# f1tenth/f1tenth_planning

Hardware: AMD Instinct MI355X
Metric: candidate-trajectory-steps/sec per GPU; p50 plan() latency @4096 egos (higher is better)
Workload: dtype f32 filter + f64 decision

## Files before the change

f1tenth_planning_amd/csrc/k_lattice_refine.hip:

```cpp
#include "lattice_mixed.h"

namespace f1p {

template <int GS>
__device__ __forceinline__ double group_shr1(double v) {
    const long long b = __double_as_longlong(v);
    const int lo = (int)(b & 0xffffffffll), hi = (int)(b >> 32);
    constexpr int ctrl = GS == 16 ? 0x111 : 0x138;
    const int slo = __builtin_amdgcn_update_dpp(0, lo, ctrl, 0xf, 0xf, false), shi = __builtin_amdgcn_update_dpp(0, hi, ctrl, 0xf, 0xf, false);
    return __longlong_as_double(((long long)shi << 32) | (long long)(unsigned int)slo);
}

template <int GS, bool FOOT = false, typename... OB>
__global__ __launch_bounds__(256, 2) void k_lattice_refine(const unsigned int* __restrict__ h_qcount, const RefEntry* __restrict__ h_q, unsigned int h_q_shard_cap, unsigned int h_grid,
                                                           LatticeArgs a, f1p_lattice_cfg cfg, MixArgs mx, OB... obx) {
    extern __shared__ __align__(16) unsigned char lds_raw[];
    constexpr bool OBS = sizeof...(OB) > 0;
    int ka[32];
    warm_kernargs_touch<24 + sizeof(LatticeArgs) + sizeof(f1p_lattice_cfg) + sizeof(MixArgs) + (sizeof(OB) + ... + 0)>(ka);
    constexpr int GPW = 64 / GS;
    constexpr unsigned int WPB = F1P_MIX_REFINE_BLOCK / 64;
    const int tid = threadIdx.x, lane = tid & 63, wave = tid >> 6;
    const int gl = lane & (GS - 1), grp = lane / GS, gbase = lane & ~(GS - 1);
    const unsigned int ngroups_total = h_grid * WPB * GPW;
    const unsigned int g0 = (blockIdx.x * WPB + wave) * GPW + grp;
    const unsigned int sh = (g0 / GPW) % F1P_MIX_QSHARDS, lstride = ngroups_total / F1P_MIX_QSHARDS;
    const unsigned int li_first = (g0 / (GPW * F1P_MIX_QSHARDS)) * GPW + g0 % GPW;
    RefEntry r_first;
    r_first.ok = 0; r_first.e = 0; r_first.c = 0; r_first.gx = 0; r_first.gy = 0; r_first.gth = 0; r_first.cost = 0; r_first.k0 = 0; r_first.dk = 0; r_first.L = 0; r_first.pad = 0;
    unsigned int n = h_qcount[sh * 32u];
    if (li_first < h_q_shard_cap) r_first = h_q[sh * h_q_shard_cap + li_first];
    warm_kernargs_wait(ka, n, r_first.ok);
    const int S_arg = cfg.n_stations;
    if (mx.perm_fill) {
        const int np = F1P_MIX_OREG * mx.perm_rs;
        for (int i = (int)(blockIdx.x * blockDim.x) + tid; i < np; i += (int)(gridDim.x * blockDim.x)) mx.perm_fill[i] = 0;
        if (blockIdx.x == 0 && tid < 2 * F1P_MIX_OREG) mx.ocnt[tid * 32u] = 0u;
    }
    __shared__ double s_gl_wu[16][6];
    __shared__ double s_gl_x[16];
#ifdef F1P_MIX_PHASES
    long long rph[16]; int nrp = 0;
#define F1P_RPH() do { if (nrp < 15) rph[nrp++] = clock64(); } while (0)
#else
#define F1P_RPH() do {} while (0)
#endif
    F1P_RPH();
    const bool collide_on = cfg.check_collision && a.has_grid;
    if (tid < 96) s_gl_wu[tid / 6][tid % 6] = c_gl_wu[tid / 6][tid % 6];
    else if (tid < 112) s_gl_x[tid - 96] = c_gl_x[tid - 96];
    __syncthreads();
    asm volatile("" : "+v"(n), "+v"(r_first.ok));
    for (unsigned int ib = 0, li = li_first; ; ib += ngroups_total, li += lstride) {
#ifdef F1P_MIX_REFINE_LICM
        const int S = S_arg;
#else
        int S = S_arg;
        asm volatile("" : "+s"(S));
#endif
        const int den = S - 1 > 1 ? S - 1 : 1;
        const int sim_m = S - cfg.n_shift - cfg.n_cull;
        double* ncs = reinterpret_cast<double*>(lds_raw) + (size_t)(wave * GPW + grp) * (64 + 4 * (size_t)S);
        double* nsn = ncs + 32;
        double* inc_x = nsn + 32;
        double* inc_y = inc_x + S;
        double* akv = inc_y + S;
        double* simv = akv + S;
        const unsigned int i = sh * mx.q_shard_cap + li;
        const bool live = li < n;
        if (!__any(live)) break;
        RefEntry r = r_first;
        if (ib != 0) {
            r.ok = 0; r.e = 0; r.c = 0; r.gx = 0; r.gy = 0; r.gth = 0; r.cost = 0; r.k0 = 0; r.dk = 0; r.L = 0; r.pad = 0;
            if (li < mx.q_shard_cap) r = mx.q[i];
        }
        if (!live) { r.ok = 0; r.e = a.e0; r.c = 0; }
        F1P_RPH();
        const bool work = live && r.ok != 0;
        const int e = r.e;
        const bool check_occ = collide_on && r.ok != -2;
        EgoXform xf = {};
        if (work && check_occ) xf = mx.xf[e];
        [[maybe_unused]] bool check_disc = false;
        [[maybe_unused]] int n_live = 0;
        [[maybe_unused]] double pace = 0.0;
        [[maybe_unused]] const double* slots = nullptr;
        if constexpr (OBS) {
            const LatObs& ob = lat_obs_arg(obx...);
            if (work && r.ok != -2) {
                n_live = ob.n_live[e]; pace = ob.pace[e]; slots = ob.xf + (size_t)e * (5 * F1P_LATTICE_MAX_OBS);
                check_disc = n_live > 0;
            }
        }
        const double* prev = a.prev_theta ? a.prev_theta + (size_t)e * S : nullptr;
        double pv[4] = {0.0, 0.0, 0.0, 0.0};
        if (work && prev) {
#pragma unroll
            for (int k = 0; k < 4; ++k) { const int q = gl + k * GS; if (q < sim_m) pv[k] = prev[q + cfg.n_shift]; }
        }
        Clothoid cl;
        cl.ok = false; cl.k0 = 0; cl.dk = 0; cl.L = 0;
        G1State g;
        g.r = 0; g.phi0 = 0; g.delta = 0; g.A = 0;
        bool fitting = work && g1_begin(r.gx, r.gy, r.gth, g);
        F1P_RPH();
        double c0 = 0.0;
        bool ok = false;
        for (int it = 0; it < 20 && __any(fitting); ++it) {
            const double fa = g.A, fb = g.delta - g.A, fc = g.phi0;
            const double exc = fabs(fa) + fabs(fb);
            int off = 88, cnt = 32, panels = 1;
            if (exc <= 8.0) { off = 0; cnt = 16; }
            else if (exc <= 14.0) { off = 16; cnt = 20; }
            else if (exc <= 21.0) { off = 36; cnt = 24; }
            else if (exc <= 29.0) { off = 60; cnt = 28; }
            else if (!(exc <= 36.0)) {
                const double pn = __builtin_ceil(exc * (1.0 / 36.0));
                panels = pn <= 1024.0 ? (int)pn : 1024;
            }
            if (!fitting) { cnt = 0; panels = 1; }
            double acc = 0.0;
            const int k = gl < 6 ? gl : gl - 6;
            int max_panels = panels;
            if (__any(panels > 1)) {
#pragma unroll
                for (int m_ = 32; m_ >= 1; m_ >>= 1) { const int o = __shfl_xor(max_panels, m_, 64); max_panels = o > max_panels ? o : max_panels; }
            }
            if (max_panels == 1) {
                const bool rule16 = cnt == 16;
                for (int j = gl; j < cnt; j += GS) {
                    const double tau = rule16 ? s_gl_x[j] : c_gl_x[off + j];
                    const double ph = __builtin_fma(__builtin_fma(fa, tau, fb), tau, fc);
                    double sn, cs;
                    sincos_core(ph, &sn, &cs);
                    ncs[j] = cs; nsn[j] = sn;
                }
                __builtin_amdgcn_s_waitcnt(0xc07f);
                __builtin_amdgcn_wave_barrier();
#ifdef F1P_MIX_PHASES
                if (it == 0) F1P_RPH();
#endif
                if (gl < 12) {
                    const double* v = gl < 6 ? ncs : nsn;
                    if (rule16) {
                        double w[16], u[16];
#pragma unroll
                        for (int j = 0; j < 16; ++j) { w[j] = s_gl_wu[j][k]; u[j] = v[j]; }
#pragma unroll
                        for (int j = 0; j < 16; ++j) acc = __builtin_fma(w[j], u[j], acc);
                    } else {
                        for (int j0 = 0; j0 < cnt; j0 += 4) {
                            const double w0 = c_gl_wu[off + j0][k], w1 = c_gl_wu[off + j0 + 1][k], w2 = c_gl_wu[off + j0 + 2][k], w3 = c_gl_wu[off + j0 + 3][k];
                            const double u0 = v[j0], u1 = v[j0 + 1], u2 = v[j0 + 2], u3 = v[j0 + 3];
                            acc = __builtin_fma(w0, u0, acc); acc = __builtin_fma(w1, u1, acc); acc = __builtin_fma(w2, u2, acc); acc = __builtin_fma(w3, u3, acc);
                        }
                    }
                }
                __builtin_amdgcn_wave_barrier();
            } else {
                const double h = 1.0 / (double)panels;
                for (int p = 0; p < max_panels; ++p) {
                    const bool mine = fitting && p < panels;
                    if (mine && panels == 1) {
                        for (int j = gl; j < cnt; j += GS) {
                            const double tau = c_gl_x[off + j];
                            const double ph = __builtin_fma(__builtin_fma(fa, tau, fb), tau, fc);
                            double sn, cs;
                            sincos_core(ph, &sn, &cs);
                            ncs[j] = cs; nsn[j] = sn;
                        }
                    } else if (mine) {
                        const double t0 = (double)p * h;
                        for (int j = gl; j < cnt; j += GS) {
                            const double tau = __builtin_fma(h, c_gl_x[off + j], t0);
                            const double ph = __builtin_fma(__builtin_fma(fa, tau, fb), tau, fc);
                            double sn, cs;
                            sincos_core(ph, &sn, &cs);
                            const double w = h * c_gl_w[off + j];
                            ncs[j] = w * cs; nsn[j] = w * sn;
                            akv[j] = __builtin_fma(tau, tau, -tau);
                        }
                    }
                    __builtin_amdgcn_s_waitcnt(0xc07f);
                    __builtin_amdgcn_wave_barrier();
                    if (mine && gl < 12) {
                        const double* v = gl < 6 ? ncs : nsn;
                        if (panels == 1) {
                            for (int j = 0; j < cnt; ++j) acc = __builtin_fma(c_gl_wu[off + j][k], v[j], acc);
                        } else {
                            for (int j = 0; j < cnt; ++j) {
                                double t = v[j];
                                for (int q = 0; q < k; ++q) t *= akv[j];
                                acc += t;
                            }
                        }
                    }
                    __builtin_amdgcn_wave_barrier();
                }
            }
            FitMoments m;
#pragma unroll
            for (int q = 0; q < 6; ++q) { m.c[q] = shfl_d(acc, gbase + q); m.s[q] = shfl_d(acc, gbase + 6 + q); }
#ifdef F1P_MIX_PHASES
            if (it == 0) F1P_RPH();
#endif
            if (fitting) {
                const int st = g1_step(m, g, c0);
                if (st != 0) { fitting = false; ok = st > 0; }
            }
        }
        if (ok) cl = g1_finish(g, c0);
        F1P_RPH();
        double cost = __builtin_huge_val();
        const bool run = cl.ok;
        const double k0 = cl.k0, dk = cl.dk, L = run ? cl.L : 1.0;
        const double ds = L / (double)den;
        bool hit = false;
        const bool occ_pass = run && (check_occ || (OBS && check_disc));
        const bool store_inc = run && mx.inc != nullptr && li < mx.inc_cap;
        const bool inc_pass = occ_pass || store_inc;
        double rix[4] = {0.0, 0.0, 0.0, 0.0}, riy[4] = {0.0, 0.0, 0.0, 0.0};
        if (__any(inc_pass)) {
            if (inc_pass) {
                const IntervalCoef ic = interval_setup(k0, dk, L, ds);
                const int per = (S - 1 + GS - 1) / GS, q0 = gl * per, q1 = q0 + per < S - 1 ? q0 + per : S - 1;
                if (!FOOT && per <= 4) {
#pragma unroll
                    for (int k = 0; k < 4; ++k) { rix[k] = 0.0; riy[k] = 0.0; }
                    if (q0 < q1) {
                        PieceState st = piece_state_at(k0, dk, ds, q0, ic);
#pragma unroll
                        for (int k = 0; k < 4; ++k) {
                            if (q0 + k < q1) interval_increment(k0, dk, (double)(q0 + k) * ds, (q0 + k) * ic.nsub, ic, st, rix[k], riy[k]);
                        }
                    }
                } else if (q0 < q1) {
                    PieceState st = piece_state_at(k0, dk, ds, q0, ic);
                    for (int q = q0; q < q1; ++q) {
                        double dx, dy;
                        interval_increment(k0, dk, (double)q * ds, q * ic.nsub, ic, st, dx, dy);
                        inc_x[q] = dx; inc_y[q] = dy;
                    }
                }
            }
            __builtin_amdgcn_s_waitcnt(0xc07f);
            __builtin_amdgcn_wave_barrier();
            F1P_RPH();
            double* gp = store_inc ? mx.inc + ((size_t)sh * mx.inc_cap + li) * 2 * (size_t)S : nullptr;
            double* pos_x = akv; double* pos_y = simv;
            if (inc_pass) {
                const int per = (S - 1 + GS - 1) / GS;
                if (gl == 0) { pos_x[0] = 0.0; pos_y[0] = 0.0; }
                if (!FOOT && per <= 4) {
                    const int nrounds = (S - 1 + per - 1) / per;
                    double xin = 0.0, yin = 0.0, xo = 0.0, yo = 0.0;
                    for (int t = 0; t < nrounds; ++t) {
                        xin = group_shr1<GS>(xo); yin = group_shr1<GS>(yo);
                        xo = xin; yo = yin;
#pragma unroll
                        for (int k = 0; k < 4; ++k) { xo += rix[k]; yo += riy[k]; }
                    }
                    double x = xin, y = yin;
                    const int q0 = gl * per;
#pragma unroll
                    for (int k = 0; k < 4; ++k) {
                        x += rix[k]; y += riy[k];
                        if (k < per && q0 + k < S - 1) { pos_x[q0 + k + 1] = x; pos_y[q0 + k + 1] = y; }
                    }
                } else {
                double x = 0.0, y = 0.0;
                int j0 = 0;
                for (; j0 + 8 <= S - 1; j0 += 8) {
                    double dx[8], dy[8], xs[8], ys[8];
#pragma unroll
                    for (int u = 0; u < 8; ++u) { dx[u] = inc_x[j0 + u]; dy[u] = inc_y[j0 + u]; }
#pragma unroll
                    for (int u = 0; u < 8; ++u) { x += dx[u]; y += dy[u]; xs[u] = x; ys[u] = y; }
                    if (gl == 0) {
#pragma unroll
                        for (int u = 0; u < 8; ++u) { pos_x[j0 + u + 1] = xs[u]; pos_y[j0 + u + 1] = ys[u]; }
                    }
                }
                for (; j0 < S - 1; ++j0) {
                    x += inc_x[j0]; y += inc_y[j0];
                    if (gl == 0) { pos_x[j0 + 1] = x; pos_y[j0 + 1] = y; }
                }
                }
            }
            __builtin_amdgcn_s_waitcnt(0xc07f);
            __builtin_amdgcn_wave_barrier();
            F1P_RPH();
            if (inc_pass) {
                constexpr int NSL = 4;
                for (int qb = 0; qb < S; qb += NSL * GS) {
                    double xs[NSL], ys[NSL];
#pragma unroll
                    for (int k = 0; k < NSL; ++k) { const int q = qb + k * GS + gl; xs[k] = q < S ? pos_x[q] : 0.0; ys[k] = q < S ? pos_y[q] : 0.0; }
                    auto cell = [&](double qx, double qy, uint32_t& word, int& bit) {
                        word = 0xffffffffu; bit = 0;
                        const double lxf = __builtin_floor(__builtin_fma(xf.txx, qx, __builtin_fma(xf.txy, qy, xf.tx0)));
                        const double lyf = __builtin_floor(__builtin_fma(xf.tyx, qx, __builtin_fma(xf.tyy, qy, xf.ty0)));
                        const double gxf = lxf + (double)xf.tile_gx0, gyf = lyf + (double)xf.tile_gy0;
                        if ((gxf >= 0.0) & (gxf < (double)a.grid.w) & (gyf >= 0.0) & (gyf < (double)a.grid.h)) {
                            const int cgx = (int)gxf, cgy = (int)gyf;
                            word = a.grid.bits[(size_t)cgy * a.grid.wwords + (cgx >> 5)];
                            bit = cgx & 31;
                        }
                    };
                    if (gp) {
#pragma unroll
                        for (int k = 0; k < NSL; ++k) { const int q = qb + k * GS + gl; if (q < S) { __builtin_nontemporal_store(xs[k], gp + q); __builtin_nontemporal_store(ys[k], gp + S + q); } }
                    }
                    if (!occ_pass) continue;
                    if constexpr (OBS) {
                        if (check_disc) {
#pragma unroll
                            for (int k = 0; k < NSL; ++k) {
                                const int q = qb + k * GS + gl;
                                if (q < S) hit |= lat_disc_blocked(slots, n_live, xs[k], ys[k], ((double)q * ds) * pace);
                            }
                        }
                        if (!check_occ) continue;
                    }
                    if (!FOOT || mx.n_disc == 0) {
                        uint32_t word[NSL]; int bit[NSL]; bool have[NSL];
#pragma unroll
                        for (int k = 0; k < NSL; ++k) {
                            have[k] = qb + k * GS + gl < S;
                            word[k] = 0u; bit[k] = 0;
                            if (have[k]) cell(xs[k], ys[k], word[k], bit[k]);
                        }
#pragma unroll
                        for (int k = 0; k < NSL; ++k) hit |= have[k] && ((word[k] >> bit[k]) & 1u);
                    } else {
#pragma unroll
                        for (int k = 0; k < NSL; ++k) {
                            const int q = qb + k * GS + gl;
                            if (q < S) {
                                const double sq = (double)q * ds;
                                const double th = sq * (k0 + 0.5 * sq * dk);
                                double sn_h, cs_h;
                                sincos_fast(th, &sn_h, &cs_h);
                                for (int d = 0; d < mx.n_disc; ++d) {
                                    const double o = mx.disc_off[d];
                                    uint32_t word; int bit;
                                    cell(xs[k] + o * cs_h, ys[k] + o * sn_h, word, bit);
                                    hit |= (word >> bit) & 1u;
                                }
                            }
                        }
                    }
                }
            }
            __builtin_amdgcn_s_waitcnt(0xc07f);
            __builtin_amdgcn_wave_barrier();
        }
        F1P_RPH();
        if (run) {
            for (int q = gl; q < S; q += GS) {
                const double s = (double)q * ds;
                akv[q] = fabs(k0 + dk * s);
                double sv = 0.0;
                if (prev && q < sim_m) {
                    const int kq = (q - gl) / GS;
                    const double pq = kq < 4 ? (kq == 0 ? pv[0] : (kq == 1 ? pv[1] : (kq == 2 ? pv[2] : pv[3]))) : prev[q + cfg.n_shift];
                    const double th = s * (k0 + 0.5 * s * dk); const double d = th - pq; sv = d * d;
                }
                simv[q] = sv;
            }
        }
        __builtin_amdgcn_s_waitcnt(0xc07f);
        __builtin_amdgcn_wave_barrier();
        F1P_RPH();
        const unsigned long long hm = __ballot(hit);
        const bool any_hit = ((hm >> gbase) & (GS == 64 ? ~0ull : (1ull << (GS & 63)) - 1ull)) != 0ull;
        if (run) {
            double sumk = 0.0, sim = 0.0;
            {
                int q = 0;
                for (; q + 8 <= S; q += 8) {
                    double v[8];
#pragma unroll
                    for (int u = 0; u < 8; ++u) v[u] = akv[q + u];
#pragma unroll
                    for (int u = 0; u < 8; ++u) sumk += v[u];
                }
                for (; q < S; ++q) sumk += akv[q];
            }
            if (prev) {
                int q = 0;
                for (; q + 8 <= sim_m; q += 8) {
                    double v[8];
#pragma unroll
                    for (int u = 0; u < 8; ++u) v[u] = simv[q + u];
#pragma unroll
                    for (int u = 0; u < 8; ++u) sim += v[u];
                }
                for (; q < sim_m; ++q) sim += simv[q];
            }
            const double maxk = __builtin_fmax(fabs(k0 + dk * (0.0 * ds)), fabs(k0 + dk * ((double)(S - 1) * ds)));
            cost = 0.0;
            cost += cfg.w_length * (1.0 / L);
            cost += cfg.w_max_kappa * maxk;
            cost += cfg.w_mean_kappa * (sumk / (double)S);
            cost += cfg.w_similarity * sim;
            if (any_hit) cost = __builtin_huge_val();
        }
        __builtin_amdgcn_wave_barrier();
        if (work && gl == 0) {
            RefEntry o = r;
            o.cost = cost; o.k0 = cl.k0; o.dk = cl.dk; o.L = cl.L; o.ok = cl.ok ? 1 : 0; o.pad = store_inc ? 1 : 0;
            mx.q[i] = o;
        }
#ifdef F1P_MIX_PHASES
        F1P_RPH();
        if (ib == 0 && live && gl == 0 && mx.dbg_state && (size_t)i * 16 + 16 <= (size_t)a.E * cfg.n_lookahead * cfg.n_width) {
            for (int k = 0; k + 1 < nrp; ++k) mx.dbg_state[(size_t)i * 16 + k] = (int)(rph[k + 1] - rph[k]);
            mx.dbg_state[(size_t)i * 16 + 15] = nrp;
        }
#endif
    }
}

template <int GS, bool FOOT = false>
__global__ __launch_bounds__(256, 2) void k_lattice_refine_cubic(LatticeArgs a, f1p_lattice_cfg cfg, MixArgs mx) {
    extern __shared__ __align__(16) unsigned char lds_raw[];
    warm_kernargs<sizeof(LatticeArgs) + sizeof(f1p_lattice_cfg) + sizeof(MixArgs)>();
    constexpr int GPW = 64 / GS;
    const int tid = threadIdx.x, lane = tid & 63, wave = tid >> 6;
    const int gl = lane & (GS - 1), grp = lane / GS, gbase = lane & ~(GS - 1);
    const int S = cfg.n_stations;
    if (mx.perm_fill) {
        const int np = F1P_MIX_OREG * mx.perm_rs;
        for (int i = (int)(blockIdx.x * blockDim.x) + tid; i < np; i += (int)(gridDim.x * blockDim.x)) mx.perm_fill[i] = 0;
        if (blockIdx.x == 0 && tid < 2 * F1P_MIX_OREG) mx.ocnt[tid * 32u] = 0u;
    }
    const bool collide_on = cfg.check_collision && a.has_grid;
    const unsigned int ngroups_total = gridDim.x * (blockDim.x >> 6) * GPW;
    const unsigned int g0 = (blockIdx.x * (blockDim.x >> 6) + wave) * GPW + grp;
    const unsigned int sh = (g0 / GPW) % F1P_MIX_QSHARDS, lstride = ngroups_total / F1P_MIX_QSHARDS;
    const unsigned int li_first = (g0 / (GPW * F1P_MIX_QSHARDS)) * GPW + g0 % GPW;
    const unsigned int n = mx.qcount[sh * 32u];
    const int den = S - 1 > 1 ? S - 1 : 1;
    const int sim_m = S - cfg.n_shift - cfg.n_cull;
    double* px = reinterpret_cast<double*>(lds_raw) + (size_t)(wave * GPW + grp) * 5 * (size_t)S;
    double* py = px + S;
    double* chv = py + S;
    double* akv = chv + S;
    double* simv = akv + S;
    for (unsigned int li = li_first; ; li += lstride) {
        const bool live = li < n;
        if (!__any(live)) break;
        const unsigned int i = sh * mx.q_shard_cap + li;
        RefEntry r;
        r.ok = 0; r.e = a.e0; r.c = 0; r.gx = 0; r.gy = 0; r.gth = 0; r.cost = 0; r.k0 = 0; r.dk = 0; r.L = 0; r.pad = 0;
        if (live) r = mx.q[i];
        const bool work = live && r.ok != 0;
        const int e = r.e;
        const bool check_occ = collide_on && r.ok != -2;
        EgoXform xf = {};
        if (work && check_occ) xf = mx.xf[e];
        const double* prev = a.prev_theta ? a.prev_theta + (size_t)e * S : nullptr;
        Cubic cq = cubic_setup(r.gx, r.gy, r.gth);
        const bool run = work && cq.ok;
        bool hit = false;
        double maxk = 0.0;
        for (int q = gl; q < S; q += GS) {
            double x = 0.0, y = 0.0, th = 0.0, ak = 0.0;
            if (run) cubic_row(cq, (double)q / (double)den, x, y, th, ak);
            px[q] = x; py[q] = y; akv[q] = ak;
            double sv = 0.0;
            if (run && prev && q < sim_m) { const double d = th - prev[q + cfg.n_shift]; sv = d * d; }
            simv[q] = sv;
            maxk = __builtin_fmax(maxk, ak);
            if (run && check_occ) {
                auto occupied = [&](double qx, double qy) -> bool {
                    uint32_t word = 0xffffffffu; int bit = 0;
                    const double lxf = __builtin_floor(__builtin_fma(xf.txx, qx, __builtin_fma(xf.txy, qy, xf.tx0)));
                    const double lyf = __builtin_floor(__builtin_fma(xf.tyx, qx, __builtin_fma(xf.tyy, qy, xf.ty0)));
                    const double gxf = lxf + (double)xf.tile_gx0, gyf = lyf + (double)xf.tile_gy0;
                    if ((gxf >= 0.0) & (gxf < (double)a.grid.w) & (gyf >= 0.0) & (gyf < (double)a.grid.h)) {
                        const int cgx = (int)gxf, cgy = (int)gyf;
                        word = a.grid.bits[(size_t)cgy * a.grid.wwords + (cgx >> 5)];
                        bit = cgx & 31;
                    }
                    return ((word >> bit) & 1u) != 0u;
                };
                if (!FOOT || mx.n_disc == 0) hit |= occupied(x, y);
                else {
                    double sn_h, cs_h;
                    sincos_fast(th, &sn_h, &cs_h);
                    for (int d = 0; d < mx.n_disc; ++d) {
                        const double o = mx.disc_off[d];
                        hit |= occupied(x + o * cs_h, y + o * sn_h);
                    }
                }
            }
        }
        __builtin_amdgcn_s_waitcnt(0xc07f);
        __builtin_amdgcn_wave_barrier();
        for (int q = gl; q < S; q += GS) {
            double ch = 0.0;
            if (q > 0) { const double ddx = px[q] - px[q - 1], ddy = py[q] - py[q - 1]; ch = __builtin_sqrt(ddx * ddx + ddy * ddy); }
            chv[q] = ch;
        }
        __builtin_amdgcn_s_waitcnt(0xc07f);
        __builtin_amdgcn_wave_barrier();
        double acc = 0.0;
        {
            const double* arr = gl == 0 ? chv : (gl == 1 ? akv : simv);
            const int cnt = gl == 2 ? (sim_m > 0 ? sim_m : 0) : S;
            int q = 0;
            for (; q + 8 <= S; q += 8) {
                double v[8];
#pragma unroll
                for (int u = 0; u < 8; ++u) v[u] = arr[q + u];
#pragma unroll
                for (int u = 0; u < 8; ++u) acc += (q + u < cnt) ? v[u] : 0.0;
            }
            for (; q < S; ++q) acc += q < cnt ? arr[q] : 0.0;
        }
#pragma unroll
        for (int m_ = GS / 2; m_ >= 1; m_ >>= 1) maxk = __builtin_fmax(maxk, shfl_xor_d(maxk, m_));
        const double len = shfl_d(acc, gbase), sumk = shfl_d(acc, gbase + 1), sim = shfl_d(acc, gbase + 2);
        const unsigned long long hm = __ballot(hit);
        const bool any_hit = ((hm >> gbase) & (GS == 64 ? ~0ull : (1ull << (GS & 63)) - 1ull)) != 0ull;
        double cost = __builtin_huge_val();
        if (run) {
            cost = 0.0;
            cost += cfg.w_length * (1.0 / len);
            cost += cfg.w_max_kappa * maxk;
            cost += cfg.w_mean_kappa * (sumk / (double)S);
            cost += cfg.w_similarity * (prev ? sim : 0.0);
            if (any_hit) cost = __builtin_huge_val();
        }
        __builtin_amdgcn_wave_barrier();
        if (work && gl == 0) {
            RefEntry o = r;
            o.cost = cost; o.k0 = r.gx; o.dk = r.gy; o.L = r.gth; o.ok = run ? 1 : 0; o.pad = 0;
            mx.q[i] = o;
        }
    }
}

bool mixed_refine_fits(f1p_ctx* ctx, int lanes, bool foot, size_t lds, bool obs) {
    if (obs) return lanes == 16 ? lds_fits(ctx, (k_lattice_refine<16, false, LatObs>), lds) : lds_fits(ctx, (k_lattice_refine<64, false, LatObs>), lds);
    if (lanes == 16) return foot ? lds_fits(ctx, (k_lattice_refine<16, true>), lds) : lds_fits(ctx, k_lattice_refine<16>, lds);
    return foot ? lds_fits(ctx, (k_lattice_refine<64, true>), lds) : lds_fits(ctx, k_lattice_refine<64>, lds);
}

bool mixed_refine_cubic_fits(f1p_ctx* ctx, size_t lds) {
    return lds_fits(ctx, k_lattice_refine_cubic<16>, lds) && lds_fits(ctx, (k_lattice_refine_cubic<16, true>), lds);
}

void mixed_launch_refine(bool cubic, int lanes, bool foot, unsigned grid, size_t lds, hipStream_t st, const LatticeArgs& a, const f1p_lattice_cfg& cfg, const MixArgs& mx,
                         const LatObs* ob) {
    const dim3 g(grid), b(F1P_MIX_REFINE_BLOCK);
    if (ob) {
        if (lanes == 16) hipLaunchKernelGGL((k_lattice_refine<16, false, LatObs>), g, b, lds, st, mx.qcount, mx.q, mx.q_shard_cap, grid, a, cfg, mx, *ob);
        else hipLaunchKernelGGL((k_lattice_refine<64, false, LatObs>), g, b, lds, st, mx.qcount, mx.q, mx.q_shard_cap, grid, a, cfg, mx, *ob);
    } else if (cubic && foot) hipLaunchKernelGGL((k_lattice_refine_cubic<16, true>), g, b, lds, st, a, cfg, mx);
    else if (cubic) hipLaunchKernelGGL(k_lattice_refine_cubic<16>, g, b, lds, st, a, cfg, mx);
    else if (lanes == 16) {
        if (foot) hipLaunchKernelGGL((k_lattice_refine<16, true>), g, b, lds, st, mx.qcount, mx.q, mx.q_shard_cap, grid, a, cfg, mx);
        else hipLaunchKernelGGL(k_lattice_refine<16>, g, b, lds, st, mx.qcount, mx.q, mx.q_shard_cap, grid, a, cfg, mx);
    } else {
        if (foot) hipLaunchKernelGGL((k_lattice_refine<64, true>), g, b, lds, st, mx.qcount, mx.q, mx.q_shard_cap, grid, a, cfg, mx);
        else hipLaunchKernelGGL(k_lattice_refine<64>, g, b, lds, st, mx.qcount, mx.q, mx.q_shard_cap, grid, a, cfg, mx);
    }
}

}
```

f1tenth_planning_amd/csrc/lattice_mixed.h:

```cpp
#pragma once
#include "lattice_device.h"

namespace f1p {

#ifndef F1P_MIX_MIN_EGOS_V3
#define F1P_MIX_MIN_EGOS_V3 1
#endif
#ifndef F1P_MIX_MARGIN_REL
#define F1P_MIX_MARGIN_REL 3.0e-5f
#endif
#ifndef F1P_MIX_MARGIN_ABS
#define F1P_MIX_MARGIN_ABS 1.0e-6f
#endif
#ifndef F1P_MIX_MACRO
#define F1P_MIX_MACRO 1
#endif
#ifndef F1P_MIX_INC_PER_EGO
#define F1P_MIX_INC_PER_EGO 4
#endif
#ifndef F1P_MIX_EXC_MAX
#define F1P_MIX_EXC_MAX 20.0f
#endif
#ifndef F1P_MIX_LOOKAHEAD_PAIRS
#define F1P_MIX_LOOKAHEAD_PAIRS 1
#endif
#ifndef F1P_MIX_FILTER_BLOCK
#define F1P_MIX_FILTER_BLOCK 256
#endif
#ifndef F1P_MIX_FILTER_WAVES
#define F1P_MIX_FILTER_WAVES 8
#endif
#ifndef F1P_MIX_FIT_UNROLL
#define F1P_MIX_FIT_UNROLL 4
#endif
#ifndef F1P_MIX_COOP_MAX
#define F1P_MIX_COOP_MAX 4
#endif
#ifndef F1P_MIX_COOP_MAX_X
#define F1P_MIX_COOP_MAX_X 24
#endif
#ifndef F1P_MIX_OREG
#define F1P_MIX_OREG 64
#endif
#ifndef F1P_MIX_HEAVY_MEMORY
#define F1P_MIX_HEAVY_MEMORY 16
#endif
#ifndef F1P_MIX_ORDER_MIN_EGOS
#define F1P_MIX_ORDER_MIN_EGOS 1024
#endif
#ifndef F1P_MIX_ROUNDS
#define F1P_MIX_ROUNDS 10
#endif
#ifndef F1P_F3_CONTRACT
#define F1P_F3_CONTRACT 1
#endif
#if F1P_F3_CONTRACT
#define F1P_F32_CONTRACT _Pragma("clang fp contract(fast)")
#else
#define F1P_F32_CONTRACT
#endif
#ifndef F1P_F3_FIT_PAIRS
#define F1P_F3_FIT_PAIRS 1
#endif
#ifndef F1P_F3_RAW_SQRT
#define F1P_F3_RAW_SQRT 1
#endif
#ifndef F1P_F3_FAST_ATAN
#define F1P_F3_FAST_ATAN 1
#endif
#ifndef F1P_MIX_F3_EGOS_PER_WG
#define F1P_MIX_F3_EGOS_PER_WG 1
#endif
#ifndef F1P_PIPE_CHUNKS
#define F1P_PIPE_CHUNKS 1
#endif
#ifndef F1P_PIPE_MIN_EGOS
#define F1P_PIPE_MIN_EGOS 2048
#endif
#ifndef F1P_MIX_EDGE0
#define F1P_MIX_EDGE0 2.0e-4f
#endif
#ifndef F1P_MIX_EDGE1
#define F1P_MIX_EDGE1 8.0e-6f
#endif
#ifndef F1P_MIX_QSHARDS
#define F1P_MIX_QSHARDS 8
#endif
#ifndef F1P_MIX_REFINE_WG_PER_CU
#define F1P_MIX_REFINE_WG_PER_CU 4
#endif
#define F1P_MIX_REFINE_BLOCK 256
#ifndef F1P_PRO2
#define F1P_PRO2 1
#endif
#ifndef F1P_PRO2_MIN_EGOS
#define F1P_PRO2_MIN_EGOS 3072
#endif
#define F1P_ST_FREE 0
#define F1P_ST_HIT 1
#define F1P_ST_UNSURE 2
#define F1P_ST_BAD 3
#define F1P_ST_PENDING 4
#define F1P_ST_PENDING2 5
#define F1P_INV_2PI_F 0.15915494309189535f

struct RefEntry {
    int32_t e, c;
    double gx, gy, gth;
    double cost, k0, dk, L;
    int32_t ok, pad;
};

struct EgoXform { double txx, txy, tx0, tyx, tyy, ty0; int tile_gx0, tile_gy0; };


struct MixArgs {
    unsigned int* qcount;
    unsigned int q_shard_cap;
    double* inc;
    unsigned int inc_cap;
    RefEntry* q;
    int32_t* ego_base;
    int32_t* ego_n;
    int32_t* ego_ni;
    struct EgoXform* xf;
    const uint32_t* clear_bits;
    int clear_r;
    float clear_ds_cap;
    int n_disc;
    double disc_off[4];
    float disc_off_f[4], disc_omax_f;
    double sim_s2, sim_s3, sim_s4;
    float margin_rel, margin_abs;
    float edge0, edge1;
    double la_slack;
    float la_slack_f;
    float* dbg_bound;
    float* dbg_cost32;
    int32_t* dbg_state;
    int32_t* perm;
    int32_t* perm_fill;
    unsigned int* ocnt;
    unsigned char* heavy;
    int perm_rs;
    int32_t* dbg_pass;
};

struct GoalFrame32 { double cx, cy, nx, ny; float gth; int ok; };

__device__ __forceinline__ int cvt_flr_i32_f32(float v) {
    int r;
    asm("v_cvt_flr_i32_f32 %0, %1" : "=v"(r) : "v"(v));
    return r;
}

struct EgoParamsF2 {
    float txx, txy, tx0, tyx, tyy, ty0;
    float w_len, w_maxk, w_meank, w_sim;
    float margin_rel, margin_abs, edge0, edge1;
    float clear_ds_cap, inv_den, inv_S, fS;
    float cells_per_m, sqrt_S;
    float inv_nw, pad0;
    const double* prev;
    double M0, M1, M2;
    int tile_w, tile_h;
    int tile_gx0, tile_gy0;
    int S, sim_m, n_shift;
    int exact_all;
};

struct CubicTab { float h10, h01, h11, pad0, d10, d01, d11, pad1, e10, e01, e11, pad2; };

struct EgoRecHdr {
    double px, py, theta, ct, st;
    EgoParamsF2 p;
};
static_assert(sizeof(EgoRecHdr) % 8 == 0, "record header must keep the fp64 arrays aligned");

__host__ __device__ inline size_t ego_rec_stride(int nl) { return (sizeof(EgoRecHdr) + (size_t)nl * (40 + sizeof(GoalFrame32)) + 15) & ~(size_t)15; }

void mixed_launch_prologue(bool two_per_wave, bool tracks, int egos, hipStream_t st, const LatticeArgs& a, const f1p_lattice_cfg& cfg, const MixArgs& mx, unsigned char* recs);
bool mixed_filter3_fits(f1p_ctx* ctx, int cr, bool foot, bool cubic, size_t lds, bool obs = false);
void mixed_launch_filter3(int cr, bool hooks, bool host_goals, bool cubic, bool foot, unsigned grid, size_t lds, hipStream_t st, const LatticeArgs& a,
                          const f1p_lattice_cfg& cfg, const MixArgs& mx, const unsigned char* recs, const LatObs* ob = nullptr);
bool mixed_refine_fits(f1p_ctx* ctx, int lanes, bool foot, size_t lds, bool obs = false);
bool mixed_refine_cubic_fits(f1p_ctx* ctx, size_t lds);
void mixed_launch_refine(bool cubic, int lanes, bool foot, unsigned grid, size_t lds, hipStream_t st, const LatticeArgs& a, const f1p_lattice_cfg& cfg, const MixArgs& mx,
                         const LatObs* ob = nullptr);
bool mixed_select_fits(f1p_ctx* ctx, bool cubic, size_t lds, bool tracks = false);
void mixed_launch_select(bool cubic, bool tracks, unsigned grid, size_t lds, hipStream_t st, const LatticeArgs& a, const f1p_lattice_cfg& cfg, const MixArgs& mx);

}
```

Baseline: 770.2 billion.

## Overlap occupancy-grid loads with cost reduction in refine kernel for short paths

```diff
diff --git a/f1tenth_planning_amd/csrc/k_lattice_refine.hip b/f1tenth_planning_amd/csrc/k_lattice_refine.hip
--- a/f1tenth_planning_amd/csrc/k_lattice_refine.hip
+++ b/f1tenth_planning_amd/csrc/k_lattice_refine.hip
@@ -220,6 +220,11 @@
         const bool store_inc = run && mx.inc != nullptr && li < mx.inc_cap;
         const bool inc_pass = occ_pass || store_inc;
         double rix[4] = {0.0, 0.0, 0.0, 0.0}, riy[4] = {0.0, 0.0, 0.0, 0.0};
+        constexpr int NSL = 4;
+        const bool early_cost = F1P_REFINE_EARLY_COST && !FOOT && !OBS && S <= NSL * GS;
+        uint32_t ow[NSL] = {0u, 0u, 0u, 0u}; int ob_[NSL] = {0, 0, 0, 0};
+        asm volatile("" :: "v"(xf.txx), "v"(xf.txy), "v"(xf.tx0), "v"(xf.tyx), "v"(xf.tyy), "v"(xf.ty0), "v"(xf.tile_gx0), "v"(xf.tile_gy0));
+        asm volatile("" :: "v"(pv[0]), "v"(pv[1]), "v"(pv[2]), "v"(pv[3]));
         if (__any(inc_pass)) {
             if (inc_pass) {
                 const IntervalCoef ic = interval_setup(k0, dk, L, ds);
@@ -290,23 +295,39 @@
             __builtin_amdgcn_s_waitcnt(0xc07f);
             __builtin_amdgcn_wave_barrier();
             F1P_RPH();
+            auto cell = [&](double qx, double qy, uint32_t& word, int& bit) {
+                word = 0xffffffffu; bit = 0;
+                const double lxf = __builtin_floor(__builtin_fma(xf.txx, qx, __builtin_fma(xf.txy, qy, xf.tx0)));
+                const double lyf = __builtin_floor(__builtin_fma(xf.tyx, qx, __builtin_fma(xf.tyy, qy, xf.ty0)));
+                const double gxf = lxf + (double)xf.tile_gx0, gyf = lyf + (double)xf.tile_gy0;
+                if ((gxf >= 0.0) & (gxf < (double)a.grid.w) & (gyf >= 0.0) & (gyf < (double)a.grid.h)) {
+                    const int cgx = (int)gxf, cgy = (int)gyf;
+                    word = a.grid.bits[(size_t)cgy * a.grid.wwords + (cgx >> 5)];
+                    bit = cgx & 31;
+                }
+            };
+            if (early_cost) {
+                double xs[NSL] = {0.0, 0.0, 0.0, 0.0}, ys[NSL] = {0.0, 0.0, 0.0, 0.0};
+                if (inc_pass) {
+#pragma unroll
+                    for (int k = 0; k < NSL; ++k) { const int q = k * GS + gl; xs[k] = q < S ? pos_x[q] : 0.0; ys[k] = q < S ? pos_y[q] : 0.0; }
+                    if (gp) {
+#pragma unroll
+                        for (int k = 0; k < NSL; ++k) { const int q = k * GS + gl; if (q < S) { __builtin_nontemporal_store(xs[k], gp + q); __builtin_nontemporal_store(ys[k], gp + S + q); } }
+                    }
+                }
+                __builtin_amdgcn_s_waitcnt(0xc07f);
+                __builtin_amdgcn_wave_barrier();
+                if (occ_pass) {
+#pragma unroll
+                    for (int k = 0; k < NSL; ++k) { if (k * GS + gl < S) cell(xs[k], ys[k], ow[k], ob_[k]); }
+                }
+            } else {
             if (inc_pass) {
-                constexpr int NSL = 4;
                 for (int qb = 0; qb < S; qb += NSL * GS) {
                     double xs[NSL], ys[NSL];
 #pragma unroll
                     for (int k = 0; k < NSL; ++k) { const int q = qb + k * GS + gl; xs[k] = q < S ? pos_x[q] : 0.0; ys[k] = q < S ? pos_y[q] : 0.0; }
-                    auto cell = [&](double qx, double qy, uint32_t& word, int& bit) {
-                        word = 0xffffffffu; bit = 0;
-                        const double lxf = __builtin_floor(__builtin_fma(xf.txx, qx, __builtin_fma(xf.txy, qy, xf.tx0)));
-                        const double lyf = __builtin_floor(__builtin_fma(xf.tyx, qx, __builtin_fma(xf.tyy, qy, xf.ty0)));
-                        const double gxf = lxf + (double)xf.tile_gx0, gyf = lyf + (double)xf.tile_gy0;
-                        if ((gxf >= 0.0) & (gxf < (double)a.grid.w) & (gyf >= 0.0) & (gyf < (double)a.grid.h)) {
-                            const int cgx = (int)gxf, cgy = (int)gyf;
-                            word = a.grid.bits[(size_t)cgy * a.grid.wwords + (cgx >> 5)];
-                            bit = cgx & 31;
-                        }
-                    };
                     if (gp) {
 #pragma unroll
                         for (int k = 0; k < NSL; ++k) { const int q = qb + k * GS + gl; if (q < S) { __builtin_nontemporal_store(xs[k], gp + q); __builtin_nontemporal_store(ys[k], gp + S + q); } }
@@ -354,6 +375,7 @@
             }
             __builtin_amdgcn_s_waitcnt(0xc07f);
             __builtin_amdgcn_wave_barrier();
+            }
         }
         F1P_RPH();
         if (run) {
@@ -372,11 +394,30 @@
         __builtin_amdgcn_s_waitcnt(0xc07f);
         __builtin_amdgcn_wave_barrier();
         F1P_RPH();
+        double sumk = 0.0, sim = 0.0;
+        if (early_cost) {
+            double acc = 0.0;
+            if (run && gl < 2) {
+                const double* src = gl == 0 ? akv : simv;
+                const int nn = gl == 0 ? S : (prev ? sim_m : 0);
+                int q = 0;
+                for (; q + 8 <= nn; q += 8) {
+                    double v[8];
+#pragma unroll
+                    for (int u = 0; u < 8; ++u) v[u] = src[q + u];
+#pragma unroll
+                    for (int u = 0; u < 8; ++u) acc += v[u];
+                }
+                for (; q < nn; ++q) acc += src[q];
+            }
+            sumk = shfl_d(acc, gbase); sim = shfl_d(acc, gbase + 1);
+#pragma unroll
+            for (int k = 0; k < NSL; ++k) hit |= ((ow[k] >> ob_[k]) & 1u) != 0u;
+        }
         const unsigned long long hm = __ballot(hit);
         const bool any_hit = ((hm >> gbase) & (GS == 64 ? ~0ull : (1ull << (GS & 63)) - 1ull)) != 0ull;
         if (run) {
-            double sumk = 0.0, sim = 0.0;
-            {
+            if (!early_cost) {
                 int q = 0;
                 for (; q + 8 <= S; q += 8) {
                     double v[8];
@@ -387,7 +428,7 @@
                 }
                 for (; q < S; ++q) sumk += akv[q];
             }
-            if (prev) {
+            if (prev && !early_cost) {
                 int q = 0;
                 for (; q + 8 <= sim_m; q += 8) {
                     double v[8];
diff --git a/f1tenth_planning_amd/csrc/lattice_mixed.h b/f1tenth_planning_amd/csrc/lattice_mixed.h
--- a/f1tenth_planning_amd/csrc/lattice_mixed.h
+++ b/f1tenth_planning_amd/csrc/lattice_mixed.h
@@ -85,6 +85,9 @@
 #endif
 #ifndef F1P_MIX_QSHARDS
 #define F1P_MIX_QSHARDS 8
+#endif
+#ifndef F1P_REFINE_EARLY_COST
+#define F1P_REFINE_EARLY_COST 1
 #endif
 #ifndef F1P_MIX_REFINE_WG_PER_CU
 #define F1P_MIX_REFINE_WG_PER_CU 4
```

Result: no change. 776.8 billion, median of 6 (+0.9%).
